# exosports/BART

Hardware: NVIDIA B200
Metric: forward_model_spectra_per_s (higher is better)
Workload: dtype f64

## Files before the change

### bart_b200/csrc/column_math.cuh

```cuda
#pragma once
#include "device.cuh"
#include <cmath>
#include <cstring>
#include <vector>

namespace bart {

constexpr double cPI = 3.141592653589793;
constexpr double cAMU = 1.66053886e-24;
constexpr double cLS = 2.99792458e10;
constexpr double cKB = 1.380658e-16;
constexpr double cH = 6.6260755e-27;
constexpr double cAMAGAT = 2.68678e19;
constexpr double cE0H2 = 4.911e-23;
constexpr double cNAVO = 6.02214076e23;
constexpr double cMICRON = 1e-4;

enum { REJ_TGRID = 1, REJ_TCIA = 2, REJ_SUMQ = 4, REJ_FEWPTS = 8, REJ_NOTOOMUCH = 64 };

BART_HD double bits_to_double(long long b) {
#ifdef __CUDA_ARCH__
  return __longlong_as_double(b);
#else
  double d; memcpy(&d, &b, 8); return d;
// ... 507 lines not shown
    }
  }
  row[L.SA] = sa;
  row[L.SB] = sb;
  row[L.SC] = scf;
  row[L.TR] = tr;
}

BART_HD int prep_table_row(const DevConfig &c, const PrepPtrs &pp, const KnobVals &kv, int d,
                           const double *temp, const double *rho, int rho_stride, const double *radius,
                           double *tab, int model = 0) {
  int status = prep_row_thermal(c, pp, d, temp, rho, rho_stride, tab, model);
  status |= prep_row_cia(c, pp, d, temp, rho, rho_stride, tab);
  prep_row_scat(c, pp, kv, d, temp, rho, rho_stride, tab);
  prep_row_radius(c, d, radius, tab);
  return status;
}
BART_HD int prep_table_row(const DevConfig &c, const KnobVals &kv, int d, const double *temp,
                           const double *rho, int rho_stride, const double *radius, double *tab,
                           int model = 0) {
  return prep_table_row(c, prep_ptrs_of(c), kv, d, temp, rho, rho_stride, radius, tab, model);
}

struct ColPtrs {
  const char *g;
  const char *cia[kMaxCia];
};
template <int NCIA>
BART_HD ColPtrs col_ptrs(const DevConfig &c, int w) {
  ColPtrs P;
  P.g = reinterpret_cast<const char *>(c.grid) + (size_t)w * c.gms * 8;
#pragma unroll
  for (int f = 0; f < (NCIA >= 0 ? NCIA : kMaxCia); f++)
    P.cia[f] = f < c.ncia ? reinterpret_cast<const char *>(c.ciaPQ[f]) + (size_t)w * 32 : nullptr;
  return P;
}

template <int NMOL, int NCIA>
struct CellData {
  static constexpr bool kStatic = NMOL >= 1 && NMOL <= 4;
  static constexpr bool kStaticCia = kStatic && NCIA >= 0;
  static constexpr int NG = !kStatic ? 1 : (NMOL == 1 ? 1 : (NMOL == 2 ? 2 : 4));
  static constexpr int NC = kStaticCia && NCIA > 0 ? NCIA : 1;
  double lo[NG], hi[NG];
  D4 q[NC];
};

template <int NCIA>
struct CellOffs {
  long long g;
  long long cia[NCIA > 0 ? NCIA : 1];
};
template <int NMOL, int NCIA>
BART_HD CellOffs<NCIA> cell_offsets(const double *row) {
  typedef TabLayout L;
  CellOffs<NCIA> o;
  o.g = double_to_bits(row[L::GOFF]);
#pragma unroll
  for (int f = 0; f < (NCIA > 0 ? NCIA : 0); f++) o.cia[f] = double_to_bits(row[L::W + 2 * NMOL + 6 * f]);
  return o;
}

template <int NMOL, int NCIA>
BART_HD void cell_load_at(const DevConfig &c, const ColPtrs &P, const CellOffs<NCIA> &o,
                          CellData<NMOL, NCIA> &x, size_t goff = 0, size_t coff = 0,
                          bool with_cia = true) {
  if (!CellData<NMOL, NCIA>::kStatic) return;
  const size_t plane = (size_t)c.nwave * c.gms * 8;
  const char *lo = P.g + o.g;
  const char *hi = lo + plane;
  if (NMOL == 1) { x.lo[0] = ldg1b(lo + goff); x.hi[0] = ldg1b(hi + goff); }
  else if (NMOL == 2) {
    const D2 a = ldg2b(lo + goff), b = ldg2b(hi + goff);
    x.lo[0] = a.x; x.lo[1] = a.y; x.hi[0] = b.x; x.hi[1] = b.y;
  } else {
    const D4 a = ld4b(lo + goff), b = ld4b(hi + goff);
    x.lo[0] = a.x; x.lo[1] = a.y; x.lo[2] = a.z; x.lo[3] = a.w;
    x.hi[0] = b.x; x.hi[1] = b.y; x.hi[2] = b.z; x.hi[3] = b.w;
  }
  if (!CellData<NMOL, NCIA>::kStaticCia || !with_cia) return;
#pragma unroll
  for (int f = 0; f < (NCIA > 0 ? NCIA : 0); f++) x.q[f] = ld4b(P.cia[f] + o.cia[f] + coff);
}

template <int NMOL, int NCIA>
BART_HD void cell_load(const DevConfig &c, const ColPtrs &P, const double *row,
                       CellData<NMOL, NCIA> &x, size_t goff = 0, size_t coff = 0) {
  if (!CellData<NMOL, NCIA>::kStatic) return;
  cell_load_at<NMOL, NCIA>(c, P, cell_offsets<NMOL, NCIA>(row), x, goff, coff);
}

template <int NMOL, int NCIA, bool SC = true>
BART_HD double cell_combine(const DevConfig &c, const ColPtrs &P, const double *row,
                            const CellData<NMOL, NCIA> &x, double wn4, int part,
                            size_t goff = 0, size_t coff = 0) {
  typedef TabLayout L;
  const int ngmol = NMOL > 0 ? NMOL : c.ngmol;
  const int ncia = NCIA >= 0 ? NCIA : c.ncia;
  constexpr bool kStatic = CellData<NMOL, NCIA>::kStatic;
  double e = 0.0;
  if (kStatic) {
#pragma unroll
    for (int m = 0; m < (kStatic ? NMOL : 0); m++) {
      const D2 wt = ld2(row + L::W + 2 * m);
      e = m == 0 ? wt.x * x.lo[0] : fma(wt.x, x.lo[m < CellData<NMOL, NCIA>::NG ? m : 0], e);
      e = fma(wt.y, x.hi[m < CellData<NMOL, NCIA>::NG ? m : 0], e);
    }
  } else {
    const size_t plane = (size_t)c.nwave * c.gms * 8;
    const char *lo = P.g + double_to_bits(row[L::GOFF]) + goff;
    const char *hi = lo + plane;
    for (int m = 0; m < ngmol; m++) {
      const D2 wt = ld2(row + L::W + 2 * m);
      e = m == 0 ? wt.x * ld1b(lo) : fma(wt.x, ld1b(lo + 8 * m), e);
      e = fma(wt.y, ld1b(hi + 8 * m), e);
    }
  }
  if (part == 1) return e;
  double ecs = 0.0;
  const double *cr = row + L::W + 2 * ngmol;
#pragma unroll
  for (int f = 0; f < (NCIA >= 0 ? NCIA : kMaxCia); f++) {
    if (f < ncia) {
      D4 q;
      if (CellData<NMOL, NCIA>::kStaticCia) q = x.q[f < CellData<NMOL, NCIA>::NC ? f : 0];
      else {
        const char *pq = P.cia[f] + double_to_bits(cr[6 * f]) + coff;
        const D2 k0 = ld2b(pq), k1 = ld2b(pq + 16);
        q.x = k0.x; q.y = k0.y; q.z = k1.x; q.w = k1.y;
      }
      const D2 cy = ld2(cr + 6 * f + 2), cz = ld2(cr + 6 * f + 4);
      double v = cy.x * q.x;
      v = fma(cy.y, q.z, v);
      v = fma(cz.x, q.y, v);
      v = fma(cz.y, q.w, v);
      if (hi_word(v) > 0) ecs += v;
    }
  }
  if (part == 2) return ecs;
  if (!SC) return e + ecs;
  const D2 sc = ld2(row + L::SCAT);
  return fma(sc.x, wn4, e) + sc.y + ecs;
}

template <int NMOL, int NCIA, bool SC = true>
BART_HD double cell_extinction(const DevConfig &c, const ColPtrs &P, const double *row, double wn4,
                               int part, size_t goff = 0, size_t coff = 0) {
  CellData<NMOL, NCIA> x;
  cell_load<NMOL, NCIA>(c, P, row, x, goff, coff);
  return cell_combine<NMOL, NCIA, SC>(c, P, row, x, wn4, part, goff, coff);
}

template <int NMOL, int NCIA, int NANG, bool KEEP, int NCOL, int SQ = -1, bool CHAIN = false,
          int CSTRIDE = 0, bool PGEN = true, bool SC = true>
BART_HD void eclipse_columns(const DevConfig &c, const double *tab, const unsigned long long *etab,
                             int w0, const bool (&valid)[NCOL],
                             double *const (&tau_keep)[NCOL], int *const (&last_keep)[NCOL],
                             double (&flux)[NCOL], bool upper = false) {
  typedef TabLayout L;
  const int nl = c.nlayer;
  const int nf = c.lay.nf();
  const int nang = NANG > 0 ? NANG : c.nang;
  const int small_hi = hi_word(c.tau_small), clamp_hi = hi_word(c.tau_clamp);
  constexpr bool kStatic = CellData<NMOL, NCIA>::kStatic;
  const size_t gstep = (size_t)CSTRIDE * (kStatic ? CellData<NMOL, NCIA>::NG : c.gms) * 8;
  const size_t cstep = (size_t)CSTRIDE * 32;
  double wn4[NCOL], c2n[NCOL];
  double er1[NCOL], er2[NCOL], S[NCOL], trap[NCOL], Dprev[NCOL], Bprev[NCOL];
  int last[NCOL];
  bool alive[NCOL];
  const ColPtrs P = col_ptrs<NCIA>(c, w0);

  auto planck = [&](const double *row, double (&B)[NCOL]) {
    double E = 0.0;
    const D2 tp = ld2(row + L::INVT);
#pragma unroll
    for (int k = 0; k < NCOL; k++) {
      double em1;
      if (CHAIN && k > 0) {
        em1 = fma(E, tp.y, -1.0);
        if (k + 1 < NCOL) E *= tp.y;
      } else {
        double it = tp.x;
        if (PGEN && it * c2n[k] > kExpYmax) it = kExpYmax / c2n[k];
        if (CHAIN) {
          E = PGEN ? exp_core5(c2n[k], it, etab, 0.0) : exp_w(c2n[k], it, etab, 0.0);
          em1 = NCOL == 1 && upper ? fma(E, tp.y, -1.0) : E - 1.0;
        } else em1 = PGEN ? exp_core5(c2n[k], it, etab, -1.0) : exp_w(c2n[k], it, etab, -1.0);
      }
      B[k] = fast_rcp1(em1);
    }
  };

#pragma unroll
  for (int k = 0; k < NCOL; k++) {
    const int wk = w0 + k * CSTRIDE;
    const double wn = c.wn[wk < c.nwave ? wk : c.nwave - 1];
    wn4[k] = (wn * wn) * (wn * wn);
    c2n[k] = cH * wn * cLS / cKB * kExpScale;
    if (CHAIN && NCOL == 1 && upper) c2n[k] = cH * c.wn[wk - CSTRIDE] * cLS / cKB * kExpScale;
    er1[k] = cell_extinction<NMOL, NCIA, SC>(c, P, tab, wn4[k], false, k * gstep, k * cstep);
    er2[k] = 0.0; S[k] = 0.0; trap[k] = 0.0; Dprev[k] = c.d0;
    alive[k] = valid[k] && !(0.0 > c.toomuch);
    last[k] = alive[k] ? nl - 1 : 0;
    if (KEEP && valid[k]) tau_keep[k][0] = 0.0;
  }
  planck(tab, Bprev);

  auto any_alive = [&]() {
    bool a = false;
#pragma unroll
    for (int k = 0; k < NCOL; k++) a = a || alive[k];
    return BART_WARP_ANY(a);
  };

  CellData<NMOL, NCIA> cur[NCOL];
  const double *row_last = tab + (size_t)(nl - 1) * nf;
  auto row_after = [&](const double *r) { return r < row_last ? r + nf : r; };
#pragma unroll
  for (int k = 0; k < NCOL; k++)
    cell_load<NMOL, NCIA>(c, P, row_after(tab), cur[k], k * gstep, k * cstep);
  CellOffs<NCIA> offs = cell_offsets<NMOL, NCIA>(row_after(row_after(tab)));
  CellOffs<NCIA> have = cell_offsets<NMOL, NCIA>(row_after(tab));

  auto step = [&](const double *row, int d, bool odd) {
    double tau[NCOL], B[NCOL], D[NCOL];
    bool small[NCOL];
    double erk[NCOL];
#pragma unroll
    for (int k = 0; k < NCOL; k++) {
      erk[k] = cell_combine<NMOL, NCIA, SC>(c, P, row, cur[k], wn4[k], false, k * gstep, k * cstep);
    }
    bool fresh = false;
#pragma unroll
    for (int f = 0; f < (NCIA > 0 ? NCIA : 0); f++) fresh = fresh || offs.cia[f] != have.cia[f];
#pragma unroll
    for (int k = 0; k < NCOL; k++) cell_load_at<NMOL, NCIA>(c, P, offs, cur[k], k * gstep, k * cstep, fresh);
    if (kStatic) { have = offs; offs = cell_offsets<NMOL, NCIA>(row_after(row_after(row))); }
#pragma unroll
    for (int k = 0; k < NCOL; k++) {
      const double er = erk[k];
      if (odd) tau[k] = fma(row[L::TR], er + er1[k], S[k]);
      else {
        const D2 s1 = ld2(row + L::SA);
        S[k] = fma(s1.x, er, fma(s1.y, er1[k], fma(row[L::SC], er2[k], S[k])));
        tau[k] = S[k];
      }
      er2[k] = er1[k]; er1[k] = er;
      small[k] = !alive[k] || hi_word(tau[k]) < small_hi;
    }
    planck(row, B);
    auto series = [&](int k0, int k1) {
#pragma unroll
      for (int k = 0; k < NCOL; k++)
        if (k >= k0 && k < k1) {
          const double u = fma(tau[k], c.ser_s, -1.0);
          double p = c.taylor[kTaylorN - 1];
#pragma unroll
          for (int i = kTaylorN - 2; i >= 0; i--) p = fma(p, u, c.taylor[i]);
          D[k] = p;
        }
    };
    auto exponentials = [&](int k0, int k1) {
      bool big = false;
      double tc[NCOL];
#pragma unroll
      for (int k = 0; k < NCOL; k++) { big = big || hi_word(tau[k]) >= clamp_hi; tc[k] = tau[k]; }
      if (BART_WARP_ANY(big)) {
#pragma unroll
        for (int k = 0; k < NCOL; k++) tc[k] = hi_word(tau[k]) >= clamp_hi ? c.tau_clamp : tau[k];
      }
      if (SQ >= 0) {
#pragma unroll
        for (int k = 0; k < NCOL; k++)
          if (k >= k0 && k < k1) {
            const double e = exp_w(tc[k], -c.exp_a[SQ >> 4], etab + (1 + (SQ >> 4)) * kExpTabSize, 0.0);
            D[k] = fma(e * e, c.sq_coef, e);
          }
      } else {
#pragma unroll
        for (int k = 0; k < NCOL; k++) if (k >= k0 && k < k1) D[k] = 0.0;
      }
#pragma unroll
      for (int a = 0; a < (NANG > 0 ? NANG : kMaxAng); a++)
        if (a < nang && !(SQ >= 0 && (a == (SQ >> 4) || a == (SQ & 15)))) {
#pragma unroll
          for (int k = 0; k < NCOL; k++)
            if (k >= k0 && k < k1) D[k] = exp_w(tc[k], -c.exp_a[a], etab + (1 + a) * kExpTabSize, D[k]);
        }
    };
    unsigned sm = 0;
#pragma unroll
    for (int k = 0; k < NCOL; k++) sm |= BART_WARP_ALL(small[k]) ? 1u << k : 0u;
    if (sm == (1u << NCOL) - 1u) series(0, NCOL);
    else if (sm == 0u) exponentials(0, NCOL);
    else {
#pragma unroll
      for (int k = 0; k < NCOL; k++) { if (sm >> k & 1u) series(k, k + 1); else exponentials(k, k + 1); }
    }
#pragma unroll
    for (int k = 0; k < NCOL; k++)
      if (alive[k]) {
        if (KEEP) tau_keep[k][d] = tau[k];
        trap[k] = fma(D[k] - Dprev[k], B[k] + Bprev[k], trap[k]);
        Dprev[k] = D[k]; Bprev[k] = B[k];
        if (tau[k] > c.toomuch) { last[k] = d; alive[k] = false; }
      }
  };

  const double *row = tab + nf;
  for (int d = 1; d < nl; d += 2, row += 2 * nf) {
    if (!any_alive()) break;
    step(row, d, true);
    if (d + 1 >= nl) break;
    step(row + nf, d + 1, false);
  }
#pragma unroll
  for (int k = 0; k < NCOL; k++) {
    if (KEEP && valid[k]) *last_keep[k] = last[k];
    const int wk = w0 + k * CSTRIDE;
    const double wn = c.wn[wk < c.nwave ? wk : c.nwave - 1];
    const double c1 = 2.0 * cH * (wn * wn * wn) * cLS * cLS;
    flux[k] = cPI * c1 * (Bprev[k] * Dprev[k] - 0.5 * trap[k]);
  }
}

template <int NMOL, int NCIA, int NANG, bool KEEP>
BART_HD double eclipse_column(const DevConfig &c, const double *tab, const unsigned long long *etab,
                              int w, double *tau_keep, int *last_keep) {
  const bool valid[1] = {true};
  double *const tk[1] = {tau_keep};
  int *const lk[1] = {last_keep};
  double flux[1];
  eclipse_columns<NMOL, NCIA, NANG, KEEP, 1>(c, tab, etab, w, valid, tk, lk, flux);
  return flux[0];
}

template <class Acc, class Rad>
BART_HD void transit_weight_row_parts(const DevConfig &c, Rad rad, int d, Acc W, int part, int nparts) {
  if (d == 0) { if (part == 0) W(0) = 0.0; return; }
  const double b = rad(d);
  const double f = 2.0 * c.rfct;
  if (d == 1) {
    if (part != 0) return;
    const double rm = (rad(1) + rad(0)) / 2.0;
    const double s1 = sqrt(rm * rm - b * b), s2 = sqrt(rad(0) * rad(0) - b * b);
    const double h0 = s1, h1 = s2 - s1;
    const double hsum = h0 + h1, hratio = h1 / h0, hfactor = hsum * hsum / (h0 * h1);
    const double a0 = (2.0 - hratio) * hsum / 6.0, a1 = hfactor * hsum / 6.0,
                 a2 = (2.0 - 1.0 / hratio) * hsum / 6.0;
    W(1) = f * (a0 + 0.5 * a1);
    W(0) = f * (a2 + 0.5 * a1);
    return;
  }
  auto sdep = [&](int i) { return i == d ? 0.0 : sqrt(rad(i) * rad(i) - b * b); };
  auto panel = [&](double sT, double sM, double sB, double &top, double &mid, double &bot) {
    const double h0 = sM - sB, h1 = sT - sM;
    const double hsum = h0 + h1, hratio = h1 / h0, hfactor = hsum * hsum / (h0 * h1);
    bot = f * (2.0 - hratio) * hsum / 6.0;
    mid = f * hfactor * hsum / 6.0;
    top = f * (2.0 - 1.0 / hratio) * hsum / 6.0;
  };
  const int P = d / 2;
  const int p0 = (int)((long long)P * part / nparts), p1 = (int)((long long)P * (part + 1) / nparts);
  const bool tail = part == nparts - 1;
  if (p0 == p1 && !tail) return;
  double sT = sdep(2 * p0), carry = 0.0;
  if (p0 > 0) {
    double t, m, bt;
    panel(sdep(2 * p0 - 2), sdep(2 * p0 - 1), sT, t, m, bt);
    carry = 0.0 + bt;
  }
  for (int p = p0; p < p1; p++) {
    const double sM = sdep(2 * p + 1), sB = sdep(2 * p + 2);
    double top, mid, bot;
    panel(sT, sM, sB, top, mid, bot);
    W(2 * p) = carry + top;
    W(2 * p + 1) = 0.0 + mid;
    carry = 0.0 + bot;
    sT = sB;
  }
  if (!tail) return;
  if (d & 1) {
    const double h = sdep(d - 1);
    W(d - 1) = carry + f * h / 2.0;
    W(d) = 0.0 + f * h / 2.0;
  } else W(d) = carry;
}
template <class Acc>
BART_HD void transit_weight_row_acc(const DevConfig &c, const double *tab, int d, Acc W, int part = 0,
                                    int nparts = 1) {
  const int nf = c.lay.nf();
  transit_weight_row_parts(c, [tab, nf](int i) { return tab[(size_t)i * nf + TabLayout::RAD]; }, d, W, part, nparts);
}

BART_HD void transit_weight_row(const DevConfig &c, const double *tab, int d, double *wt) {
  transit_weight_row_acc(c, tab, d, [wt](int i) -> double & { return wt[i]; });
}

constexpr int kTrChunk = 20, kTrTD = 5, kTrGroup = 6, kTrRow = (kTrChunk / kTrTD) * kTrGroup;
BART_HD int tr_rows(int nl, int ch) { const int r = kTrChunk * (ch + 1); return r < nl ? r : nl; }
BART_HD size_t tr_chunk_off(int nl, int ch) {
  size_t rows = 0;
  for (int k = 0; k < ch; k++) rows += tr_rows(nl, k);
// ... 90 lines not shown
```

### bart_b200/csrc/kernels.cu

```cuda
#include "column_math.cuh"
#include "kernels.hpp"
#include <cuda_runtime.h>
#include <cstring>
#include <cstdlib>
#include <algorithm>

namespace bart {

__device__ __forceinline__ uint32_t smem_u32(const void *p) {
  return (uint32_t)__cvta_generic_to_shared(p);
}
__device__ __forceinline__ void mbar_init(uint64_t *bar, uint32_t count) {
  asm volatile("mbarrier.init.shared::cta.b64 [%0], %1;" ::"r"(smem_u32(bar)), "r"(count) : "memory");
}
__device__ __forceinline__ void fence_mbar_init() {
  asm volatile("fence.mbarrier_init.release.cluster;" ::: "memory");
  asm volatile("fence.proxy.async.shared::cta;" ::: "memory");
}
__device__ __forceinline__ void mbar_expect_tx(uint64_t *bar, uint32_t bytes) {
  asm volatile("mbarrier.arrive.expect_tx.shared::cta.b64 _, [%0], %1;" ::"r"(smem_u32(bar)), "r"(bytes)
               : "memory");
}
__device__ __forceinline__ void bulk_g2s(void *dst, const void *src, uint32_t bytes, uint64_t *bar) {
  asm volatile(
      "cp.async.bulk.shared::cluster.global.mbarrier::complete_tx::bytes [%0], [%1], %2, [%3];" ::"r"(
          smem_u32(dst)),
      "l"(src), "r"(bytes), "r"(smem_u32(bar))
      : "memory");
}
__device__ __forceinline__ void mbar_arrive(uint64_t *bar) {
  asm volatile("mbarrier.arrive.shared::cta.b64 _, [%0];" ::"r"(smem_u32(bar)) : "memory");
}
__device__ __forceinline__ void mbar_wait(uint64_t *bar, uint32_t parity) {
  uint32_t ok;
  do {
    asm volatile(
        "{\n\t.reg .pred p;\n\t"
        "mbarrier.try_wait.parity.shared::cta.b64 p, [%1], %2;\n\t"
        "selp.u32 %0, 1, 0, p;\n\t}"
        : "=r"(ok)
        : "r"(smem_u32(bar)), "r"(parity)
        : "memory");
  } while (!ok);
}

__device__ unsigned long long g_exp_table[(1 + kMaxAng) * kExpTabSize];

__device__ __forceinline__ void stage_table(double *s_tab, const double *g_tab, int ndoubles,
                                            uint64_t *bar, bool use_tma,
                                            unsigned long long *s_etab = nullptr,
                                            int n_etab = kExpTabSize) {
  if (s_etab)
    for (int j = threadIdx.x; j < n_etab; j += blockDim.x) s_etab[j] = g_exp_table[j];
  if (use_tma) {
    if (threadIdx.x == 0) { mbar_init(bar, 1); fence_mbar_init(); }
    __syncthreads();
    if (threadIdx.x == 0) {
      const uint32_t bytes = (uint32_t)ndoubles * 8u;
      mbar_expect_tx(bar, bytes);
      uint32_t off = 0;
      while (off < bytes) {
        uint32_t n = bytes - off;
        if (n > 65536u) n = 65536u;
        bulk_g2s((char *)s_tab + off, (const char *)g_tab + off, n, bar);
        off += n;
      }
    }
    mbar_wait(bar, 0);
    if (s_etab) __syncthreads();
  } else {
    for (int i = threadIdx.x; i < ndoubles; i += blockDim.x) s_tab[i] = g_tab[i];
    __syncthreads();
  }
}

constexpr int kPrepThreads = 256;
__host__ __device__ inline size_t atm_prep_smem_doubles(const DevConfig &c) {
  size_t n = ((size_t)c.nspec + 3) * c.nlayer;
  n += ((size_t)c.nspec + 1) * c.nlayer;
  n += (size_t)c.nlayer + c.ntemp + 2 * (size_t)c.nspec;
  for (int f = 0; f < c.ncia; f++) n += c.cia_nt[f];
  n += (size_t)c.lay.stride();
  return n + 8;
}
__global__ void __launch_bounds__(kPrepThreads)
atm_prep_kernel(DevConfig c, Knobs knobs, const double *__restrict__ profiles, int n_in,
                double *__restrict__ tabs, int *__restrict__ status,
                const int *__restrict__ pre_status, int nmodels, int staged) {
  extern __shared__ __align__(128) unsigned char smem_raw[];
  const int m = blockIdx.x;
  if (m >= nmodels) return;
  if (pre_status && pre_status[m] != 0) {
    if (threadIdx.x == 0) status[m] = pre_status[m];
    return;
  }
  const int nl = c.nlayer;
  double *s_rho = reinterpret_cast<double *>(smem_raw);
  double *s_mu = s_rho + (size_t)c.nspec * nl;
  double *s_rad = s_mu + nl;
  double *s_hc = s_rad + nl;
  __shared__ int s_status;
  if (threadIdx.x == 0) s_status = 0;
  const double *in = profiles + (size_t)m * n_in;
  double *tab = tabs + (size_t)m * c.lay.stride();
  const double *s_in = in;
  double *s_tabrec = tab;
  PrepPtrs pp = prep_ptrs_of(c);
  if (staged) {
    double *w_in = s_hc + nl;
    double *s_press = w_in + ((size_t)c.nspec + 1) * nl;
    double *s_gtemp = s_press + nl;
    double *s_mass = s_gtemp + c.ntemp;
    double *s_pol = s_mass + c.nspec;
    double *s_ciaT = s_pol + c.nspec;
    const int nprof = (c.nspec + 1) * nl;
    for (int i = threadIdx.x; i < nprof; i += blockDim.x) w_in[i] = in[i];
    for (int i = threadIdx.x; i < nl; i += blockDim.x) s_press[i] = c.press[i];
    for (int i = threadIdx.x; i < c.ntemp; i += blockDim.x) s_gtemp[i] = c.gtemp[i];
    for (int i = threadIdx.x; i < c.nspec; i += blockDim.x) { s_mass[i] = c.mass[i]; s_pol[i] = c.pol ? c.pol[i] : 0.0; }
    double *dst = s_ciaT;
#pragma unroll
    for (int f = 0; f < kMaxCia; f++)
      if (f < c.ncia) {
        for (int i = threadIdx.x; i < c.cia_nt[f]; i += blockDim.x) dst[i] = c.ciaT[f][i];
        pp.ciaT[f] = dst;
        dst += c.cia_nt[f];
      }
    pp.press = s_press; pp.gtemp = s_gtemp; pp.mass = s_mass; pp.pol = s_pol;
    s_in = w_in;
    s_tabrec = dst + ((reinterpret_cast<uintptr_t>(dst) & 8) ? 1 : 0);
  }
  __syncthreads();
  int st = 0;
  for (int i = threadIdx.x; i < c.nspec * nl; i += blockDim.x) {
    const int j = i / nl, l = i - j * nl;
    s_rho[i] = prep_density(c, pp, s_in, l, j);
  }
  for (int l = threadIdx.x; l < nl; l += blockDim.x) st |= prep_mu(c, pp, s_in, l, s_mu + l);
  __syncthreads();
  const KnobVals kv = knobs_for(knobs, m);
  for (int l = threadIdx.x; l < nl - 1; l += blockDim.x) s_hc[l] = hydro_coef(c, pp, s_in, s_mu, l);
  __syncthreads();
  if (knobs.radius_file) {
    for (int l = threadIdx.x; l < nl; l += blockDim.x) s_rad[l] = knobs.radius_file[l];
  } else if (threadIdx.x == 0 || threadIdx.x == 32)
    hydrostatic_radii(c, pp, kv.r0, s_in, s_mu, s_hc, s_rad, threadIdx.x == 0 ? 1 : 2);
  {
    const int first = knobs.radius_file ? 0 : 64;
    const int nthr = (int)blockDim.x - first;
    if ((int)threadIdx.x >= first)
      for (int i = (int)threadIdx.x - first; i < 3 * nl; i += nthr) {
        const int part = i / nl, d = i - part * nl;
        if (part == 0) st |= prep_row_thermal(c, pp, d, s_in, s_rho, nl, s_tabrec, c.lbl_model0 + m);
        else if (part == 1) st |= prep_row_cia(c, pp, d, s_in, s_rho, nl, s_tabrec);
        else prep_row_scat(c, pp, kv, d, s_in, s_rho, nl, s_tabrec);
      }
  }
  __syncthreads();
  for (int d = threadIdx.x; d < nl; d += blockDim.x) prep_row_radius(c, d, s_rad, s_tabrec);
  if (c.lbl)
    for (int i = threadIdx.x; i < nl * c.nspec; i += blockDim.x) {
      const int l = i / c.nspec, j = i - l * c.nspec;
      c.lbl_dens[((size_t)(c.lbl_model0 + m) * nl + l) * c.nspec + j] = s_rho[(size_t)j * nl + l];
    }
  if (st) atomicOr(&s_status, st);
  __syncthreads();
  if (staged) {
    const int nd = c.lay.stride();
    for (int i = threadIdx.x; i < nd; i += blockDim.x) tab[i] = s_tabrec[i];
  }
  if (threadIdx.x == 0) status[m] = s_status;
}

template <int NMOL, int NCIA, int NANG, bool KEEP, int SQ, bool SC>
__global__ void __launch_bounds__(kEclThreads, 8)
eclipse_column_kernel(DevConfig c, const double *__restrict__ tabs, const int *__restrict__ status,
                      double *__restrict__ spectra, double *__restrict__ tau_keep,
                      int *__restrict__ last_keep, int nmodels, int use_tma) {
  extern __shared__ __align__(128) unsigned char smem_raw[];
  __shared__ __align__(8) uint64_t bar;
  unsigned long long *s_etab = reinterpret_cast<unsigned long long *>(smem_raw);
  const int n_etab = ecl_tab_entries(NANG > 0 ? NANG : c.nang);
  double *s_tab = reinterpret_cast<double *>(s_etab + n_etab);
  const int m = blockIdx.x % nmodels;
  const int tile = blockIdx.x / nmodels;
  const int w0 = tile * (kEclThreads * kEclCols) + threadIdx.x;
  const int nd = c.lay.stride();
  double *out = spectra + (size_t)m * c.nwave;
  if (status[m] != 0) {
#pragma unroll
    for (int k = 0; k < kEclCols; k++)
      if (w0 + k * kEclThreads < c.nwave) out[w0 + k * kEclThreads] = -1.0;
    return;
  }
  stage_table(s_tab, tabs + (size_t)m * nd, nd, &bar, use_tma != 0, s_etab, n_etab);
  bool valid[kEclCols];
  double *tk[kEclCols];
  int *lk[kEclCols];
  double flux[kEclCols];
#pragma unroll
  for (int k = 0; k < kEclCols; k++) {
    const int wk = w0 + k * kEclThreads;
    valid[k] = wk < c.nwave;
    const int wc = min(wk, c.nwave - 1);
    tk[k] = KEEP ? tau_keep + ((size_t)m * c.nwave + wc) * c.nlayer : nullptr;
    lk[k] = KEEP ? last_keep + (size_t)m * c.nwave + wc : nullptr;
  }
  eclipse_columns<NMOL, NCIA, NANG, KEEP, kEclCols, SQ, true, kEclThreads, NMOL == 0, SC>(c, s_tab, s_etab, w0,
                                                                                         valid, tk, lk, flux);
#pragma unroll
  for (int k = 0; k < kEclCols; k++)
    if (valid[k]) out[w0 + k * kEclThreads] = flux[k];
}

template <int NMOL, int NCIA, int NANG, int SQ, bool SC>
__global__ void __launch_bounds__(32)
eclipse_slot_kernel(DevConfig c, const double *__restrict__ tabs, const int *__restrict__ status,
                    double *__restrict__ spectra, int nmodels, int use_tma) {
  extern __shared__ __align__(128) unsigned char smem_raw[];
  __shared__ __align__(8) uint64_t bar;
  unsigned long long *s_etab = reinterpret_cast<unsigned long long *>(smem_raw);
  const int n_etab = ecl_tab_entries(NANG > 0 ? NANG : c.nang);
  double *s_tab = reinterpret_cast<double *>(s_etab + n_etab);
  const int m = blockIdx.x % nmodels;
  const int slot = blockIdx.x / nmodels;
  const int w = slot * 32 + threadIdx.x;
  const int nd = c.lay.stride();
  double *out = spectra + (size_t)m * c.nwave;
  if (status[m] != 0) {
    if (w < c.nwave) out[w] = -1.0;
    return;
  }
  stage_table(s_tab, tabs + (size_t)m * nd, nd, &bar, use_tma != 0, s_etab, n_etab);
  const bool upper = c.planck_cols > 0 && ((slot * 32) % (kEclThreads * kEclCols)) >= kEclThreads;
  const bool valid[1] = {w < c.nwave};
  double *tk[1] = {nullptr};
  int *lk[1] = {nullptr};
  double flux[1];
  eclipse_columns<NMOL, NCIA, NANG, false, 1, SQ, true, kEclThreads, NMOL == 0, SC>(c, s_tab, s_etab, w, valid, tk,
                                                                                    lk, flux, upper);
  if (valid[0]) out[w] = flux[0];
}

constexpr int kScanThreads = 128;
constexpr int kScanCols = 4;
constexpr int kScanDepths = 32 / kScanCols;
constexpr long long kScanMaxColumns = 40000;
template <int NMOL, int NCIA, int NANG, int SQ, bool SC>
__device__ __forceinline__ double eclipse_scan_columns(const DevConfig &c, const double *tab,
                                                       const unsigned long long *etab, int w0, int lane) {
  typedef TabLayout L;
  const unsigned FULL = 0xffffffffu;
  const int nl = c.nlayer, nf = c.lay.nf();
  const int nang = NANG > 0 ? NANG : c.nang;
  const int small_hi = hi_word(c.tau_small);
  const int col = lane & (kScanCols - 1), dl = lane / kScanCols;
  const int w = min(w0 + col, c.nwave - 1);
  const double wn = c.wn[w];
  const double wn4 = (wn * wn) * (wn * wn);
  const double c2n = cH * wn * cLS / cKB * kExpScale;
  const ColPtrs P = col_ptrs<NCIA>(c, w);
  const bool odd = dl & 1;
  const int top = (kScanDepths - 1) * kScanCols + col;
  double s_carry = 0.0;
  double er_p = 0.0, d_p = c.d0, b_p = 0.0;
  double trap = 0.0, BL = 0.0, DL = 0.0;
  bool done = false;
  const int nround = (nl + kScanDepths - 1) / kScanDepths;
  CellData<NMOL, NCIA> x;
  cell_load<NMOL, NCIA>(c, P, tab + (size_t)min(dl, nl - 1) * nf, x);
  for (int r = 0; r < nround; r++) {
    const int d = r * kScanDepths + dl;
    const bool live = d < nl;
    const double *row = tab + (size_t)(live ? d : nl - 1) * nf;
    const double er = cell_combine<NMOL, NCIA, SC>(c, P, row, x, wn4, 0);
    cell_load<NMOL, NCIA>(c, P, tab + (size_t)min(d + kScanDepths, nl - 1) * nf, x);
    const double B = fast_rcp1(exp_w(c2n, row[L::INVT], etab, -1.0));
    const D2 s1 = ld2(row + L::SA);
    const D2 s2 = ld2(row + L::SC);
    const double e1 = __shfl_sync(FULL, dl == kScanDepths - 1 ? er_p : er, (lane - kScanCols) & 31);
    const double e2 = __shfl_sync(FULL, dl >= kScanDepths - 2 ? er_p : er, (lane - 2 * kScanCols) & 31);
    double v = (!odd && d >= 2 && live) ? fma(s1.x, er, fma(s1.y, e1, s2.x * e2)) : 0.0;
#pragma unroll
    for (int s = 1; s < kScanDepths; s <<= 1) {
      const double t = __shfl_up_sync(FULL, v, s * kScanCols);
      if (dl >= s) v += t;
    }
    const double S = s_carry + v;
    double tau = odd ? fma(s2.y, er + e1, S) : S;
    if (d == 0) tau = 0.0;
    const bool cross = !done && live && (d >= 1 ? tau > c.toomuch : 0.0 > c.toomuch);
    const unsigned bal = (__ballot_sync(FULL, cross) >> col) & 0x11111111u;
    const int first = bal ? (__ffs(bal) - 1) / kScanCols : kScanDepths;
    const bool use = !done && live && d >= 1 && dl <= first;
    double D = c.d0;
    if (use) {
      if (hi_word(tau) < small_hi) {
        const double u = fma(tau, c.ser_s, -1.0);
        double p = c.taylor[kTaylorN - 1];
#pragma unroll
        for (int i = kTaylorN - 2; i >= 0; i--) p = fma(p, u, c.taylor[i]);
        D = p;
      } else {
        const double tc = tau < c.tau_clamp ? tau : c.tau_clamp;
        if (SQ >= 0) {
          const double e = exp_w(tc, -c.exp_a[SQ >> 4], etab + (1 + (SQ >> 4)) * kExpTabSize, 0.0);
          D = fma(e * e, c.sq_coef, e);
        } else D = 0.0;
#pragma unroll
        for (int a = 0; a < (NANG > 0 ? NANG : kMaxAng); a++)
          if (a < nang && !(SQ >= 0 && (a == (SQ >> 4) || a == (SQ & 15))))
            D = exp_w(tc, -c.exp_a[a], etab + (1 + a) * kExpTabSize, D);
      }
    }
    const double Dm = __shfl_sync(FULL, dl == kScanDepths - 1 ? d_p : D, (lane - kScanCols) & 31);
    const double Bm = __shfl_sync(FULL, dl == kScanDepths - 1 ? b_p : B, (lane - kScanCols) & 31);
    if (use) trap = fma(D - Dm, B + Bm, trap);
    const bool ends = !done && (bal != 0u || r == nround - 1);
    const int f = (bal ? first : (nl - 1) % kScanDepths) * kScanCols + col;
    const double bf = __shfl_sync(FULL, B, f), df = __shfl_sync(FULL, D, f);
    if (ends) { BL = bf; DL = df; done = true; }
    if (__all_sync(FULL, done)) break;
    s_carry += __shfl_sync(FULL, v, top);
    er_p = er; d_p = D; b_p = B;
  }
#pragma unroll
  for (int s = 16; s >= kScanCols; s >>= 1) trap += __shfl_xor_sync(FULL, trap, s);
  const double c1 = 2.0 * cH * (wn * wn * wn) * cLS * cLS;
  return cPI * c1 * (BL * DL - 0.5 * trap);
}

template <int NMOL, int NCIA, int NANG, int SQ, bool SC>
__global__ void __launch_bounds__(kScanThreads, 6)
eclipse_scan_kernel(DevConfig c, const double *__restrict__ tabs, const int *__restrict__ status,
                    double *__restrict__ spectra, int nmodels, int use_tma, int tasks_per_warp) {
  extern __shared__ __align__(128) unsigned char smem_raw[];
  __shared__ __align__(8) uint64_t bar;
  unsigned long long *s_etab = reinterpret_cast<unsigned long long *>(smem_raw);
  const int n_etab = ecl_tab_entries(NANG > 0 ? NANG : c.nang);
  double *s_tab = reinterpret_cast<double *>(s_etab + n_etab);
  constexpr int kWarps = kScanThreads / 32;
  const int m = blockIdx.x % nmodels;
  const int tile = blockIdx.x / nmodels;
  const int per = kWarps * tasks_per_warp * kScanCols;
  const int wbase = tile * per;
  const int nd = c.lay.stride();
  double *out = spectra + (size_t)m * c.nwave;
  if (status[m] != 0) {
    for (int i = threadIdx.x; i < per; i += blockDim.x)
      if (wbase + i < c.nwave) out[wbase + i] = -1.0;
    return;
  }
  stage_table(s_tab, tabs + (size_t)m * nd, nd, &bar, use_tma != 0, s_etab, n_etab);
  const int warp = threadIdx.x >> 5, lane = threadIdx.x & 31;
  for (int j = 0; j < tasks_per_warp; j++) {
    const int w0 = wbase + (j * kWarps + warp) * kScanCols;
    if (w0 >= c.nwave) break;
    const double flux = eclipse_scan_columns<NMOL, NCIA, NANG, SQ, SC>(c, s_tab, s_etab, w0, lane);
    if (lane < kScanCols && w0 + lane < c.nwave) out[w0 + lane] = flux;
  }
}

// ... 581 lines not shown
  if (threadIdx.x == 0) {
    bandflux[idx] = rejected ? -1.0 : 0.5 * ((s_part[0] + s_part[1]) + (s_part[2] + s_part[3]));
    s_copier = 0;
    if (po.world > 0) {
      __threadfence();
      const int grp = m / kPeerGroup;
      const int in_grp = (min((grp + 1) * kPeerGroup, (int)gridDim.x) - grp * kPeerGroup) * nfilters;
      if (atomicAdd(po.grpcnt + grp, 1u) == (unsigned)in_grp - 1) { s_copier = 1; __threadfence(); }
    }
  }
  __syncthreads();
  if (!s_copier) return;
  {
    const int grp = m / kPeerGroup;
    const size_t lo = (size_t)grp * kPeerGroup * nfilters;
    const size_t hi = (size_t)min((grp + 1) * kPeerGroup, (int)gridDim.x) * nfilters;
    const size_t slot = (size_t)(*po.gen & 1ull) * po.world * po.cap + (size_t)po.rank * po.cap;
    for (size_t i = lo + threadIdx.x; i < hi; i += blockDim.x) {
      const double v = __ldcg(bandflux + i);
      for (int r = 0; r < po.world; r++) po.win[r][slot + i] = v;
    }
    __threadfence_system();
    __syncthreads();
    if (threadIdx.x == 0) {
      po.grpcnt[grp] = 0;
      const unsigned int ngrp = (gridDim.x + kPeerGroup - 1) / kPeerGroup;
      if (atomicAdd(po.done, 1u) == ngrp - 1) {
        *po.done = 0;
        peer_announce(po);
      }
    }
  }
}

__global__ void peer_signal_kernel(PeerOut po) { peer_announce(po); }

__global__ void __launch_bounds__(256)
peer_wait_copy_kernel(const double *__restrict__ win, unsigned long long *flags,
                      unsigned long long *gen, int world, long long cap, long long count,
                      double *__restrict__ out, int *err, unsigned int *finished,
                      unsigned long long timeout_ns) {
  __shared__ int s_bad;
  const unsigned long long g = *gen;
  if (threadIdx.x == 0) s_bad = 0;
  __syncthreads();
  if (threadIdx.x < world) {
    const unsigned long long t0 = global_ns();
    while (ld_acquire_sys(flags + threadIdx.x) < g + 1) {
      if (global_ns() - t0 > timeout_ns) { s_bad = 1; break; }
      __nanosleep(200);
    }
  }
  __syncthreads();
  if (s_bad) { if (threadIdx.x == 0) *err = 1; }
  const double *src = win + (size_t)(g & 1ull) * world * cap;
  const long long total = (long long)world * count;
  for (long long i = blockIdx.x * (long long)blockDim.x + threadIdx.x; i < total;
       i += (long long)gridDim.x * blockDim.x) {
    const long long r = i / count, k = i - r * count;
    out[i] = __ldcg(src + r * cap + k);
  }
  __syncthreads();
  if (threadIdx.x == 0) {
    __threadfence();
    if (atomicAdd(finished, 1u) == gridDim.x - 1) { *finished = 0; __threadfence(); *gen = g + 1; }
  }
}

__global__ void fill_kernel(double *p, size_t n, double v) {
  for (size_t i = blockIdx.x * (size_t)blockDim.x + threadIdx.x; i < n; i += (size_t)gridDim.x * blockDim.x)
    p[i] = v;
}

static size_t table_smem(const DevConfig &c) {
  return ((size_t)c.lay.stride() + kExpTabSize) * sizeof(double);
}

void upload_exp_table(const DevConfig &c, cudaStream_t s) {
  unsigned long long h[(1 + kMaxAng) * kExpTabSize] = {};
  fill_ecl_exp_table(c, h);
  cudaMemcpyToSymbolAsync(g_exp_table, h, sizeof(h), 0, cudaMemcpyHostToDevice, s);
  cudaStreamSynchronize(s);
}

static size_t eclipse_smem(const DevConfig &c) {
  return ((size_t)c.lay.stride() + ecl_tab_entries(c.nang)) * sizeof(double);
}
static size_t transit_tile_smem(const DevConfig &c) {
  return table_smem(c) + ((size_t)c.nlayer * (kTrRow + kTrW) + (size_t)2 * kTrChunk * kTrW) * sizeof(double);
}

void launch_grid_relayout(const double *in, double *out, int ncells, int nmol, int gms, int nwave,
                          cudaStream_t s) {
  grid_relayout_kernel<<<148 * 8, 256, 0, s>>>(in, out, ncells, nmol, gms, nwave);
}

void launch_atm_prep(const DevConfig &c, const Knobs &k, const double *profiles, int n_in,
                     double *tabs, int *status, const int *pre_status, int nmodels,
                     cudaStream_t s) {
  size_t smem = atm_prep_smem_doubles(c) * sizeof(double);
  const int staged = smem <= 160 * 1024;
  if (!staged) smem = ((size_t)c.nspec + 3) * c.nlayer * sizeof(double);
  static size_t configured = 0;
  if (smem > 48 * 1024 && smem > configured) {
    if (cudaFuncSetAttribute(atm_prep_kernel, cudaFuncAttributeMaxDynamicSharedMemorySize, (int)smem) != cudaSuccess)
      return;
    configured = smem;
  }
  atm_prep_kernel<<<nmodels, kPrepThreads, smem, s>>>(c, k, profiles, n_in, tabs, status, pre_status, nmodels, staged);
}

template <int NMOL, int NCIA, int NANG, int SQ, bool SC>
static void launch_eclipse_scan(const DevConfig &c, const double *tabs, const int *status, double *spectra,
                                int nmodels, int use_tma, size_t smem, cudaStream_t s) {
  static size_t configured = 0;
  if (smem > 48 * 1024 && smem > configured) {
    cudaFuncSetAttribute(eclipse_scan_kernel<NMOL, NCIA, NANG, SQ, SC>,
                         cudaFuncAttributeMaxDynamicSharedMemorySize, (int)smem);
    configured = smem;
  }
  constexpr int kWarps = kScanThreads / 32;
  const long long tasks = ((long long)(c.nwave + kScanCols - 1) / kScanCols) * nmodels;
  int tpw = (int)((tasks + 148LL * 6 * kWarps - 1) / (148LL * 6 * kWarps));
  tpw = tpw < 1 ? 1 : (tpw > 8 ? 8 : tpw);
  const int per = kWarps * tpw * kScanCols;
  const int tiles = (c.nwave + per - 1) / per;
  eclipse_scan_kernel<NMOL, NCIA, NANG, SQ, SC><<<(unsigned)((size_t)tiles * nmodels), kScanThreads, smem, s>>>(
      c, tabs, status, spectra, nmodels, use_tma, tpw);
}

template <int NMOL, int NCIA, int NANG, bool KEEP, int SQ = -1, bool SC = true>
static void launch_eclipse_t(const DevConfig &c, const double *tabs, const int *status,
                             double *spectra, double *tau_keep, int *last_keep, int nmodels,
                             int use_tma, int small, cudaStream_t s) {
  const size_t smem = eclipse_smem(c);
  if constexpr (!KEEP && CellData<NMOL, NCIA>::kStaticCia) {
    if (small == 2) {
      launch_eclipse_scan<NMOL, NCIA, NANG, SQ, SC>(c, tabs, status, spectra, nmodels, use_tma, smem, s);
      return;
    }
  }
  if (small && !KEEP) {
    static size_t configured_s = 0;
    if (smem > 48 * 1024 && smem > configured_s) {
      cudaFuncSetAttribute(eclipse_slot_kernel<NMOL, NCIA, NANG, SQ, SC>,
                           cudaFuncAttributeMaxDynamicSharedMemorySize, (int)smem);
      configured_s = smem;
    }
    const int nslots = (c.nwave + 31) / 32;
    eclipse_slot_kernel<NMOL, NCIA, NANG, SQ, SC><<<(unsigned)((size_t)nslots * nmodels), 32, smem, s>>>(
        c, tabs, status, spectra, nmodels, use_tma);
    return;
  }
  static size_t configured = 0;
  if (smem > 48 * 1024 && smem > configured) {
    cudaFuncSetAttribute(eclipse_column_kernel<NMOL, NCIA, NANG, KEEP, SQ, SC>,
                         cudaFuncAttributeMaxDynamicSharedMemorySize, (int)smem);
    configured = smem;
  }
  const int per = kEclThreads * kEclCols;
  const int tiles = (c.nwave + per - 1) / per;
  eclipse_column_kernel<NMOL, NCIA, NANG, KEEP, SQ, SC>
      <<<(unsigned)((size_t)tiles * nmodels), kEclThreads, smem, s>>>(
          c, tabs, status, spectra, tau_keep, last_keep, nmodels, use_tma);
}

template <int NMOL, int NCIA, bool SC>
static void launch_eclipse_nang(const DevConfig &c, const double *tabs, const int *status,
                                double *spectra, int nmodels, int use_tma, int small, cudaStream_t s) {
  if (c.nang == 5 && c.sq_src == 0 && c.sq_dst == 3)
    launch_eclipse_t<NMOL, NCIA, 5, false, 0x03, SC>(c, tabs, status, spectra, nullptr, nullptr, nmodels, use_tma, small, s);
  else launch_eclipse_t<NMOL, NCIA, 0, false, -1, SC>(c, tabs, status, spectra, nullptr, nullptr, nmodels, use_tma, small, s);
}

template <int NMOL, bool SC>
static void launch_eclipse_ncia(const DevConfig &c, const double *tabs, const int *status,
                                double *spectra, int nmodels, int use_tma, int small, cudaStream_t s) {
  switch (c.ncia) {
    case 0: launch_eclipse_nang<NMOL, 0, SC>(c, tabs, status, spectra, nmodels, use_tma, small, s); break;
    case 1: launch_eclipse_nang<NMOL, 1, SC>(c, tabs, status, spectra, nmodels, use_tma, small, s); break;
    case 2: launch_eclipse_nang<NMOL, 2, SC>(c, tabs, status, spectra, nmodels, use_tma, small, s); break;
    default: launch_eclipse_t<0, -1, 0, false>(c, tabs, status, spectra, nullptr, nullptr, nmodels, use_tma, small, s);
  }
}

template <bool SC>
static void launch_eclipse_nmol(const DevConfig &c, const double *tabs, const int *status,
                                double *spectra, int nmodels, int use_tma, int small, cudaStream_t s) {
  switch (c.ngmol) {
    case 1: launch_eclipse_ncia<1, SC>(c, tabs, status, spectra, nmodels, use_tma, small, s); break;
    case 2: launch_eclipse_ncia<2, SC>(c, tabs, status, spectra, nmodels, use_tma, small, s); break;
    case 3: launch_eclipse_ncia<3, SC>(c, tabs, status, spectra, nmodels, use_tma, small, s); break;
    case 4: launch_eclipse_ncia<4, SC>(c, tabs, status, spectra, nmodels, use_tma, small, s); break;
    default: launch_eclipse_t<0, -1, 0, false>(c, tabs, status, spectra, nullptr, nullptr, nmodels, use_tma, small, s);
  }
}

int eclipse_small_mode(const DevConfig &c, int nmodels) {
  const char *e = getenv("BART_ECL_SMALL");
  if (e && *e) return atoi(e);
  if ((long long)c.nwave * nmodels <= kScanMaxColumns) return 2;
  const long long nslots = (c.nwave + 31) / 32;
  return nslots * nmodels <= 8LL * 148 ? 1 : 0;
}

static size_t dyn_smem_max(const void *kern) {
  int dev = 0, optin = 0;
  cudaFuncAttributes a{};
  if (cudaGetDevice(&dev) != cudaSuccess ||
      cudaDeviceGetAttribute(&optin, cudaDevAttrMaxSharedMemoryPerBlockOptin, dev) != cudaSuccess ||
      cudaFuncGetAttributes(&a, kern) != cudaSuccess) {
    cudaGetLastError();
    return 0;
  }
  return (size_t)optin > a.sharedSizeBytes ? (size_t)optin - a.sharedSizeBytes : 0;
}

static size_t eclipse_dyn_max() {
  static const size_t v = std::min({dyn_smem_max((const void *)eclipse_column_kernel<0, -1, 0, true, -1, true>),
                                    dyn_smem_max((const void *)eclipse_column_kernel<0, -1, 0, false, -1, true>),
                                    dyn_smem_max((const void *)eclipse_slot_kernel<0, -1, 0, -1, true>)});
  return v;
}
static size_t transit_tile_dyn_max() {
  static const size_t v = std::min(dyn_smem_max((const void *)transit_tile_kernel<0, -1, true>),
                                   dyn_smem_max((const void *)transit_tile_kernel<0, -1, false>));
  return v;
}

bool column_smem_fits(const DevConfig &c) {
  if (c.eclipse) return eclipse_smem(c) <= eclipse_dyn_max();
  return tr_nchunks(c.nlayer) <= kTrMaxChunks && transit_tile_smem(c) <= transit_tile_dyn_max();
}

int column_layer_limit(const DevConfig &c) {
  DevConfig t = c;
  int best = 0;
  for (int nl = 1;; nl++) {
    t.nlayer = t.lay.nl = nl;
    if (!column_smem_fits(t)) return best;
    best = nl;
  }
}

bool launch_eclipse(const DevConfig &c, const double *tabs, const int *status, double *spectra,
                    double *tau_keep, int *last_keep, int nmodels, bool keep, bool sc, int use_tma,
                    cudaStream_t s) {
  if (!column_smem_fits(c)) return false;
  if (keep) {
    launch_eclipse_t<0, -1, 0, true>(c, tabs, status, spectra, tau_keep, last_keep, nmodels, use_tma, 0, s);
    return true;
  }
  const int small = eclipse_small_mode(c, nmodels);
  if (c.planck_generic) {
    launch_eclipse_t<0, -1, 0, false>(c, tabs, status, spectra, nullptr, nullptr, nmodels, use_tma, small, s);
    return true;
  }
  if (sc) launch_eclipse_nmol<true>(c, tabs, status, spectra, nmodels, use_tma, small, s);
  else launch_eclipse_nmol<false>(c, tabs, status, spectra, nmodels, use_tma, small, s);
  return true;
}

void launch_merge_status(int *status, const int *status_col, int nmodels, cudaStream_t s) {
  merge_status_kernel<<<(nmodels + 255) / 256, 256, 0, s>>>(status, status_col, nmodels);
}

size_t transit_weights_stride(int nlayer) { return std::max(tr_stride(nlayer), mm_stride(nlayer)); }

static size_t transit_mma_smem(const DevConfig &c) {
  const int nch = mm_nchunks(c.nlayer);
  return table_smem(c) + ((size_t)kMmChunk * mm_rs(nch - 1) + (size_t)nch * kMmChunk * kMmW +
                          (size_t)2 * kMmChunk * kMmW) * sizeof(double);
}
bool transit_uses_mma(const DevConfig &c, bool keep) {
  if (keep) return false;
  if (const char *e = getenv("BART_TRANSIT_MMA")) { if (*e && atoi(e) == 0) return false; }
  return mm_nchunks(c.nlayer) <= kMmMaxChunks && transit_mma_smem(c) <= 200 * 1024;
}

template <int NMOL, int NCIA, bool KEEP>
static void launch_transit_t(const DevConfig &c, const double *tabs, const double *wts,
                             const int *status, int *status_col, double *spectra, double *tau_keep,
                             int *last_keep, int nmodels, int use_tma, cudaStream_t s) {
  const size_t smem = transit_tile_smem(c);
  static size_t configured = 0;
  if (smem > 48 * 1024 && smem > configured) {
    cudaFuncSetAttribute(transit_tile_kernel<NMOL, NCIA, KEEP>,
                         cudaFuncAttributeMaxDynamicSharedMemorySize, (int)smem);
    configured = smem;
  }
  const int tiles = (c.nwave + kTrW - 1) / kTrW;
  transit_tile_kernel<NMOL, NCIA, KEEP><<<(unsigned)((size_t)tiles * nmodels), kTrThreads, smem, s>>>(
      c, tabs, wts, status, status_col, spectra, tau_keep, last_keep, nmodels, use_tma);
}

template <int NMOL, int NCIA, bool SC>
static void launch_transit_mma_sc(const DevConfig &c, const double *tabs, const double *wts,
                                  const int *status, int *status_col, double *spectra, int nmodels,
                                  int use_tma, cudaStream_t s) {
  const size_t smem = transit_mma_smem(c);
  static size_t configured = 0;
  if (smem > 48 * 1024 && smem > configured) {
    cudaFuncSetAttribute(transit_mma_kernel<NMOL, NCIA, false, SC>, cudaFuncAttributeMaxDynamicSharedMemorySize, (int)smem);
    configured = smem;
  }
  const int tiles = (c.nwave + kMmW - 1) / kMmW;
  transit_mma_kernel<NMOL, NCIA, false, SC><<<(unsigned)((size_t)tiles * nmodels), kMmThreads, smem, s>>>(
      c, tabs, wts, status, status_col, spectra, nullptr, nullptr, nmodels, use_tma);
}
static bool g_transit_sc = true;
template <int NMOL, int NCIA>
static void launch_transit_mma_t(const DevConfig &c, const double *tabs, const double *wts,
                                 const int *status, int *status_col, double *spectra, int nmodels,
                                 int use_tma, cudaStream_t s) {
  if (g_transit_sc) launch_transit_mma_sc<NMOL, NCIA, true>(c, tabs, wts, status, status_col, spectra, nmodels, use_tma, s);
  else launch_transit_mma_sc<NMOL, NCIA, false>(c, tabs, wts, status, status_col, spectra, nmodels, use_tma, s);
}

template <int NMOL>
static void launch_transit_ncia(const DevConfig &c, const double *tabs, const double *wts,
                                const int *status, int *status_col, double *spectra, int nmodels,
                                int use_tma, cudaStream_t s) {
  if (transit_uses_mma(c, false)) {
    switch (c.ncia) {
      case 0: launch_transit_mma_t<NMOL, 0>(c, tabs, wts, status, status_col, spectra, nmodels, use_tma, s); return;
      case 1: launch_transit_mma_t<NMOL, 1>(c, tabs, wts, status, status_col, spectra, nmodels, use_tma, s); return;
      case 2: launch_transit_mma_t<NMOL, 2>(c, tabs, wts, status, status_col, spectra, nmodels, use_tma, s); return;
      default: launch_transit_mma_t<0, -1>(c, tabs, wts, status, status_col, spectra, nmodels, use_tma, s); return;
    }
  }
  switch (c.ncia) {
    case 0: launch_transit_t<NMOL, 0, false>(c, tabs, wts, status, status_col, spectra, nullptr, nullptr, nmodels, use_tma, s); break;
    case 1: launch_transit_t<NMOL, 1, false>(c, tabs, wts, status, status_col, spectra, nullptr, nullptr, nmodels, use_tma, s); break;
    case 2: launch_transit_t<NMOL, 2, false>(c, tabs, wts, status, status_col, spectra, nullptr, nullptr, nmodels, use_tma, s); break;
    default: launch_transit_t<0, -1, false>(c, tabs, wts, status, status_col, spectra, nullptr, nullptr, nmodels, use_tma, s);
  }
}

void launch_transit_weights(const DevConfig &c, const double *tabs, double *wts, int nmodels,
                            bool keep, int *status_col, cudaStream_t s) {
  transit_weights_kernel<<<nmodels, kTwThreads, (size_t)c.nlayer * sizeof(double), s>>>(
      c, tabs, wts, nmodels, transit_uses_mma(c, keep) ? 1 : 0, status_col);
}

bool launch_transit(const DevConfig &c, const double *tabs, const double *wts, const int *status,
                    int *status_col, double *spectra, double *tau_keep, int *last_keep,
                    int nmodels, bool keep, bool sc, int use_tma, cudaStream_t s) {
  if (!column_smem_fits(c)) return false;
  g_transit_sc = sc;
  if (keep) {
    launch_transit_t<0, -1, true>(c, tabs, wts, status, status_col, spectra, tau_keep, last_keep, nmodels, use_tma, s);
    return true;
  }
  switch (c.ngmol) {
    case 1: launch_transit_ncia<1>(c, tabs, wts, status, status_col, spectra, nmodels, use_tma, s); break;
    case 2: launch_transit_ncia<2>(c, tabs, wts, status, status_col, spectra, nmodels, use_tma, s); break;
    case 3: launch_transit_ncia<3>(c, tabs, wts, status, status_col, spectra, nmodels, use_tma, s); break;
    case 4: launch_transit_ncia<4>(c, tabs, wts, status, status_col, spectra, nmodels, use_tma, s); break;
    default:
      if (transit_uses_mma(c, false)) launch_transit_mma_t<0, -1>(c, tabs, wts, status, status_col, spectra, nmodels, use_tma, s);
      else launch_transit_t<0, -1, false>(c, tabs, wts, status, status_col, spectra, nullptr, nullptr, nmodels, use_tma, s);
  }
  return true;
}

void launch_extinction(const DevConfig &c, const double *tabs, double *ext, int nmodels,
                       int mol_only, int layer_splits, int use_tma, cudaStream_t s) {
  const size_t smem = (size_t)c.lay.stride() * sizeof(double);
  const int tiles = (c.nwave + kColThreads - 1) / kColThreads;
  dim3 grid((unsigned)((size_t)tiles * nmodels), (unsigned)layer_splits);
  auto go = [&](auto kern) {
    if (smem > 48 * 1024)
      cudaFuncSetAttribute(kern, cudaFuncAttributeMaxDynamicSharedMemorySize, (int)smem);
// ... 41 lines not shown
```

Baseline: 938,900.

## Add non-prefetch eclipse path with fewer live registers and higher occupancy bound

Adds an AHEAD template switch to the eclipse column loop. With it off, each layer's cell data is loaded inside the step instead of being prefetched one layer ahead. The trapezoid/Simpson accumulation is reformulated so the er2 history register is dropped, and the kernel's minimum blocks per SM rises from 8 to 10 for static, low-CIA, non-keep cases. The host keeps the prefetching variant only for small grids and uses the lower-register variant otherwise, trading latency hiding for occupancy.

After: 1.018 million (median of 6 runs). 8.5% higher.

```diff
diff --git a/bart_b200/csrc/column_math.cuh b/bart_b200/csrc/column_math.cuh
--- a/bart_b200/csrc/column_math.cuh
+++ b/bart_b200/csrc/column_math.cuh
@@ -683,7 +683,7 @@
 }
 
 template <int NMOL, int NCIA, int NANG, bool KEEP, int NCOL, int SQ = -1, bool CHAIN = false,
-          int CSTRIDE = 0, bool PGEN = true, bool SC = true>
+          int CSTRIDE = 0, bool PGEN = true, bool SC = true, bool AHEAD = true>
 BART_HD void eclipse_columns(const DevConfig &c, const double *tab, const unsigned long long *etab,
                              int w0, const bool (&valid)[NCOL],
                              double *const (&tau_keep)[NCOL], int *const (&last_keep)[NCOL],
@@ -697,7 +697,7 @@
   const size_t gstep = (size_t)CSTRIDE * (kStatic ? CellData<NMOL, NCIA>::NG : c.gms) * 8;
   const size_t cstep = (size_t)CSTRIDE * 32;
   double wn4[NCOL], c2n[NCOL];
-  double er1[NCOL], er2[NCOL], S[NCOL], trap[NCOL], Dprev[NCOL], Bprev[NCOL];
+  double er1[NCOL], S[NCOL], trap[NCOL], Dprev[NCOL], Bprev[NCOL];
   int last[NCOL];
   bool alive[NCOL];
   const ColPtrs P = col_ptrs<NCIA>(c, w0);
@@ -730,8 +730,7 @@
     wn4[k] = (wn * wn) * (wn * wn);
     c2n[k] = cH * wn * cLS / cKB * kExpScale;
     if (CHAIN && NCOL == 1 && upper) c2n[k] = cH * c.wn[wk - CSTRIDE] * cLS / cKB * kExpScale;
-    er1[k] = cell_extinction<NMOL, NCIA, SC>(c, P, tab, wn4[k], false, k * gstep, k * cstep);
-    er2[k] = 0.0; S[k] = 0.0; trap[k] = 0.0; Dprev[k] = c.d0;
+    S[k] = 0.0; trap[k] = 0.0; Dprev[k] = c.d0;
     alive[k] = valid[k] && !(0.0 > c.toomuch);
     last[k] = alive[k] ? nl - 1 : 0;
     if (KEEP && valid[k]) tau_keep[k][0] = 0.0;
@@ -746,41 +745,60 @@
   };
 
   CellData<NMOL, NCIA> cur[NCOL];
+  CellOffs<NCIA> have = cell_offsets<NMOL, NCIA>(tab);
+  auto fetch = [&](const CellOffs<NCIA> &o) {
+    bool fresh = false;
+#pragma unroll
+    for (int f = 0; f < (NCIA > 0 ? NCIA : 0); f++) fresh = fresh || o.cia[f] != have.cia[f];
+#pragma unroll
+    for (int k = 0; k < NCOL; k++) cell_load_at<NMOL, NCIA>(c, P, o, cur[k], k * gstep, k * cstep, fresh);
+    have = o;
+  };
+#pragma unroll
+  for (int k = 0; k < NCOL; k++) cell_load<NMOL, NCIA>(c, P, tab, cur[k], k * gstep, k * cstep);
+#pragma unroll
+  for (int k = 0; k < NCOL; k++)
+    er1[k] = cell_combine<NMOL, NCIA, SC>(c, P, tab, cur[k], wn4[k], false, k * gstep, k * cstep);
   const double *row_last = tab + (size_t)(nl - 1) * nf;
   auto row_after = [&](const double *r) { return r < row_last ? r + nf : r; };
-#pragma unroll
-  for (int k = 0; k < NCOL; k++)
-    cell_load<NMOL, NCIA>(c, P, row_after(tab), cur[k], k * gstep, k * cstep);
-  CellOffs<NCIA> offs = cell_offsets<NMOL, NCIA>(row_after(row_after(tab)));
-  CellOffs<NCIA> have = cell_offsets<NMOL, NCIA>(row_after(tab));
+  constexpr bool kLoadInStep = kStatic && !AHEAD;
+  CellOffs<NCIA> offs;
+  if (AHEAD) {
+    fetch(cell_offsets<NMOL, NCIA>(row_after(tab)));
+    offs = cell_offsets<NMOL, NCIA>(row_after(row_after(tab)));
+  }
 
   auto step = [&](const double *row, int d, bool odd) {
     double tau[NCOL], B[NCOL], D[NCOL];
     bool small[NCOL];
     double erk[NCOL];
+    if (kLoadInStep) {
+      fetch(cell_offsets<NMOL, NCIA>(row));
+      planck(row, B);
+    }
 #pragma unroll
     for (int k = 0; k < NCOL; k++) {
       erk[k] = cell_combine<NMOL, NCIA, SC>(c, P, row, cur[k], wn4[k], false, k * gstep, k * cstep);
     }
-    bool fresh = false;
-#pragma unroll
-    for (int f = 0; f < (NCIA > 0 ? NCIA : 0); f++) fresh = fresh || offs.cia[f] != have.cia[f];
-#pragma unroll
-    for (int k = 0; k < NCOL; k++) cell_load_at<NMOL, NCIA>(c, P, offs, cur[k], k * gstep, k * cstep, fresh);
-    if (kStatic) { have = offs; offs = cell_offsets<NMOL, NCIA>(row_after(row_after(row))); }
+    if (AHEAD && kStatic) {
+      fetch(offs);
+      offs = cell_offsets<NMOL, NCIA>(row_after(row_after(row)));
+    }
 #pragma unroll
     for (int k = 0; k < NCOL; k++) {
       const double er = erk[k];
-      if (odd) tau[k] = fma(row[L::TR], er + er1[k], S[k]);
-      else {
-        const D2 s1 = ld2(row + L::SA);
-        S[k] = fma(s1.x, er, fma(s1.y, er1[k], fma(row[L::SC], er2[k], S[k])));
+      if (odd) {
+        tau[k] = fma(row[L::TR], er + er1[k], S[k]);
+        const double *nx = row_after(row);
+        S[k] = fma(nx[L::SB], er, fma(nx[L::SC], er1[k], S[k]));
+      } else {
+        S[k] = fma(row[L::SA], er, S[k]);
         tau[k] = S[k];
+        er1[k] = er;
       }
-      er2[k] = er1[k]; er1[k] = er;
       small[k] = !alive[k] || hi_word(tau[k]) < small_hi;
     }
-    planck(row, B);
+    if (!kLoadInStep) planck(row, B);
     auto series = [&](int k0, int k1) {
 #pragma unroll
       for (int k = 0; k < NCOL; k++)
diff --git a/bart_b200/csrc/kernels.cu b/bart_b200/csrc/kernels.cu
--- a/bart_b200/csrc/kernels.cu
+++ b/bart_b200/csrc/kernels.cu
@@ -4,6 +4,7 @@
 #include <cstring>
 #include <cstdlib>
 #include <algorithm>
+#include <type_traits>
 
 namespace bart {
 
@@ -172,8 +173,8 @@
   if (threadIdx.x == 0) status[m] = s_status;
 }
 
-template <int NMOL, int NCIA, int NANG, bool KEEP, int SQ, bool SC>
-__global__ void __launch_bounds__(kEclThreads, 8)
+template <int NMOL, int NCIA, int NANG, bool KEEP, int SQ, bool SC, bool AHEAD>
+__global__ void __launch_bounds__(kEclThreads, CellData<NMOL, NCIA>::kStaticCia && NCIA <= 1 && !KEEP && !AHEAD ? 10 : 8)
 eclipse_column_kernel(DevConfig c, const double *__restrict__ tabs, const int *__restrict__ status,
                       double *__restrict__ spectra, double *__restrict__ tau_keep,
                       int *__restrict__ last_keep, int nmodels, int use_tma) {
@@ -206,8 +207,8 @@
     tk[k] = KEEP ? tau_keep + ((size_t)m * c.nwave + wc) * c.nlayer : nullptr;
     lk[k] = KEEP ? last_keep + (size_t)m * c.nwave + wc : nullptr;
   }
-  eclipse_columns<NMOL, NCIA, NANG, KEEP, kEclCols, SQ, true, kEclThreads, NMOL == 0, SC>(c, s_tab, s_etab, w0,
-                                                                                         valid, tk, lk, flux);
+  eclipse_columns<NMOL, NCIA, NANG, KEEP, kEclCols, SQ, true, kEclThreads, NMOL == 0, SC, AHEAD>(
+      c, s_tab, s_etab, w0, valid, tk, lk, flux);
 #pragma unroll
   for (int k = 0; k < kEclCols; k++)
     if (valid[k]) out[w0 + k * kEclThreads] = flux[k];
@@ -1095,17 +1096,25 @@
         c, tabs, status, spectra, nmodels, use_tma);
     return;
   }
-  static size_t configured = 0;
-  if (smem > 48 * 1024 && smem > configured) {
-    cudaFuncSetAttribute(eclipse_column_kernel<NMOL, NCIA, NANG, KEEP, SQ, SC>,
-                         cudaFuncAttributeMaxDynamicSharedMemorySize, (int)smem);
-    configured = smem;
-  }
   const int per = kEclThreads * kEclCols;
   const int tiles = (c.nwave + per - 1) / per;
-  eclipse_column_kernel<NMOL, NCIA, NANG, KEEP, SQ, SC>
-      <<<(unsigned)((size_t)tiles * nmodels), kEclThreads, smem, s>>>(
-          c, tabs, status, spectra, tau_keep, last_keep, nmodels, use_tma);
+  auto launch = [&](auto ahead) {
+    const auto kern = eclipse_column_kernel<NMOL, NCIA, NANG, KEEP, SQ, SC, decltype(ahead)::value>;
+    static size_t configured = 0;
+    if (smem > 48 * 1024 && smem > configured) {
+      cudaFuncSetAttribute(kern, cudaFuncAttributeMaxDynamicSharedMemorySize, (int)smem);
+      configured = smem;
+    }
+    kern<<<(unsigned)((size_t)tiles * nmodels), kEclThreads, smem, s>>>(c, tabs, status, spectra, tau_keep,
+                                                                       last_keep, nmodels, use_tma);
+  };
+  if constexpr (CellData<NMOL, NCIA>::kStatic) {
+    if ((long long)tiles * nmodels <= 8LL * 148) {
+      launch(std::true_type());
+      return;
+    }
+  }
+  launch(std::false_type());
 }
 
 template <int NMOL, int NCIA, bool SC>
@@ -1160,8 +1169,8 @@
 }
 
 static size_t eclipse_dyn_max() {
-  static const size_t v = std::min({dyn_smem_max((const void *)eclipse_column_kernel<0, -1, 0, true, -1, true>),
-                                    dyn_smem_max((const void *)eclipse_column_kernel<0, -1, 0, false, -1, true>),
+  static const size_t v = std::min({dyn_smem_max((const void *)eclipse_column_kernel<0, -1, 0, true, -1, true, false>),
+                                    dyn_smem_max((const void *)eclipse_column_kernel<0, -1, 0, false, -1, true, false>),
                                     dyn_smem_max((const void *)eclipse_slot_kernel<0, -1, 0, -1, true>)});
   return v;
 }
```
